# samson6460/tf2_YOLO

Hardware: AMD Instinct MI355X
Metric: images/sec training YOLOv3 416x416 bs=32/GPU (higher is better)
Workload: dtype f32-storage/fp16x2-mfma

## Files before the change

### include/yolo_hip.h

```cpp
#ifndef YOLO_HIP_H_
#define YOLO_HIP_H_

#include <stddef.h>
#include <stdint.h>

#ifdef __cplusplus
extern "C" {
#endif

typedef enum yolo_status {
  YOLO_OK = 0,
  YOLO_ERR_INVALID_ARG = -1,
  YOLO_ERR_LAUNCH = -2,
  YOLO_ERR_WORKSPACE = -3
} yolo_status;

enum { YOLO_ACT_LINEAR = 0, YOLO_ACT_LEAKY = 1, YOLO_ACT_MISH = 2 };
enum { YOLO_HEAD_V3 = 3, YOLO_HEAD_V2 = 2, YOLO_HEAD_V1 = 1, YOLO_HEAD_V4 = 4 };
enum { YOLO_NMS_HARD = 1, YOLO_NMS_SOFT = 2, YOLO_NMS_DIOU = 3 };

const char* yolo_last_error(void);
int yolo_abi_version(void);
int yolo_device_available(void);
int yolo_mfma_probe(const void* operands_f16, float* sink, int workgroups, int iters, double* flops_host, void* stream);

enum { YOLO_OPT_CONV_WIN = 0, YOLO_OPT_STAMPS = 1, YOLO_OPT_CONV_SK = 2, YOLO_OPT_CONV_PATCH = 5, YOLO_OPT_WGRAD_WIN = 6,
       YOLO_OPT_NMS_WALK = 7 ,
       YOLO_OPT_AB = 8  };
int yolo_set_option(int key, int value);
size_t yolo_conv_workspace_bytes(void);
int yolo_set_conv_workspace(void* p, size_t bytes, void* stream);
int yolo_set_debug_buffer(void* p, size_t bytes);

typedef struct yolo_conv_desc {
  int N, H, W, Cin;
  int Cout, kh, kw;
  int Ho, Wo;
  int sh, sw;
  int pad_t, pad_l;
} yolo_conv_desc;

#define YOLO_BN_STAT_SLOTS 64
#define YOLO_BN_RED_SLOTS 512
#define YOLO_SPLIT_BATCH_UNITS 4

int yolo_conv2d_fwd(const yolo_conv_desc* d, const float* x, const float* w,
                    const float* bias, float* y, double* stats, void* stream);
int yolo_conv2d_fwd_absmax(const yolo_conv_desc* d, const float* x, const float* w, const float* bias,
                           float* y, double* stats, unsigned* absmax, void* stream);

int yolo_conv2d_dgrad(const yolo_conv_desc* d, const float* dy, const float* wT,
// ... 237 lines not shown
```

### tf2_yolo_amd/csrc/conv_args.hpp

```cpp
#pragma once
#include "common.hpp"

namespace yolo {

constexpr int MAX_TAPS = 49;

struct Tap {
  int oy, ox, woff;
};

struct ClassGeom {
  long long M;
  int Hg, Wg, ooy, oox, tap0, ntaps;
};

struct GatherConvArgs {
  const float* src;
  const float* wgt;
  const float* bias;
  float* dst;
  double* stats;
  unsigned* absmax;
  long long M;
  int N, Hs, Ws, Cs;
// ... 7 lines not shown
  int tiles_n;
  int nblocks;
  unsigned src_bytes, wgt_bytes;
  int zero_blk_src, zero_blk_wgt;
  int nt_store;
  int vec_store;
  int kc;
  int dbg;
  const float* epi_scale;
  const float* epi_shift;
  const float* epi_res;
  int epi_act;
  unsigned char* out_planes;
  const float* pl_pred;
  const unsigned* pl_in_bound;
  const unsigned* pl_res_bound;
  int pl_in_n, pl_res_n;
  unsigned* pl_out_words;
  float* head_y;
  const float* head_anchors;
  int head_A, head_C;
  int sk_grid;
  int tile_order;
  float* sk_slabs;
  unsigned* sk_tickets;
  int split_parts;
  int ncls;
  ClassGeom cls[4];
  unsigned long long* stamps;
  const float* bwd_y;
  const float* bwd_scale;
  const float* bwd_shift;
  const float* bwd_mean;
  const float* bwd_invstd;
  float* bwd_part;
  unsigned* bwd_aux;
  int bwd_act;
  int bwd_nslots;
  int bwd_cap;
  Tap taps[MAX_TAPS];
};

#define YOLO_BNRED_CHECK(a)                                                                                          \
  if ((a).bwd_y != nullptr && (a).bwd_nslots > (a).bwd_cap) {                                                        \
    set_error("conv_dgrad(bn reduce): %d partial slots needed, room for %d", (a).bwd_nslots, (a).bwd_cap);           \
    return YOLO_ERR_INVALID_ARG;                                                                                     \
// ... 29 lines not shown

int launch_gather_split(GatherConvArgs& a, hipStream_t st);
bool gather_split_supported(const GatherConvArgs& a);
long long planes_bytes(long long rows, int C);
int launch_split_planes(const float* x, long long rows, int C, void* planes, hipStream_t st);
int launch_split_planes_absmax(const float* x, long long rows, int C, const unsigned* absmax, const float* extra_bound, int extra_n,
                               void* planes, float* out_bound, hipStream_t st);
int launch_split_planes_concat(const float* const* xs, const int* Cs, const float* const* bounds, int nsrc, long long rows,
                               void* planes, float* dst32, float* out_bound, hipStream_t st,
                               const int* bound_words = nullptr, const int* upsample = nullptr, int H = 0, int W = 0);
int launch_split_planes_padded(const float* x, long long rows, int Csrc, int C, void* planes, hipStream_t st);
int launch_split_planes_batch(const void* jobs, int njobs, long long total_blocks, hipStream_t st);
int launch_filter_transpose_batch(const void* jobs, int njobs, long long total_blocks, hipStream_t st);
int launch_gather_planes(GatherConvArgs& a, hipStream_t st);
bool conv_small_supported(const GatherConvArgs& a);
bool conv_small_head_supported(const GatherConvArgs& a);
int launch_conv_small(GatherConvArgs& a, hipStream_t st, int* nwg);
bool gather_planes_supported(const GatherConvArgs& a);
int conv_split_parts(const GatherConvArgs& a, long long nb, int bm, int min_cb, int idle_div);
int launch_split_reduce(GatherConvArgs& a, int bm, hipStream_t st);
float* conv_split_slabs();
int launch_conv_win(GatherConvArgs& a, int variant, hipStream_t st);
bool conv_win_supported(const GatherConvArgs& a);
enum { OPT_CONV_WIN = 0, OPT_STAMPS = 1, OPT_CONV_SK = 2, OPT_DBG = 3, OPT_TILE_ORDER = 4, OPT_CONV_PATCH = 5, OPT_WGRAD_WIN = 6, OPT_NMS_WALK = 7, OPT_EXP = 8, OPT_COUNT = 16 };
int set_conv_workspace(void* p, size_t bytes, hipStream_t st);
extern void* g_dbg_buf;
extern size_t g_dbg_bytes;
extern int g_opt[OPT_COUNT];
void init_options();
int launch_wgrad_planes(WgradArgs& a, hipStream_t st);
bool wgrad_planes_supported(const WgradArgs& a);
int launch_wgrad_win(WgradArgs& a, hipStream_t st);
bool wgrad_win_supported(const WgradArgs& a);
constexpr size_t WGRAD_WS_COLSUM_BYTES = 1 << 20;
void* wgrad_workspace(size_t* bytes);
bool stem_fwd_supported(const yolo_conv_desc* d);
struct StemEpiArgs {
  const float* scale;
  const float* shift;
  int act;
  void* planes;
  const float* pred;
  const unsigned* in_words;
  int in_n;
  unsigned* out_words;
};
bool stem_infer_supported(const yolo_conv_desc* d);
// ... 15 lines not shown
```

### tf2_yolo_amd/csrc/conv_win.hip

```cpp
#include "planes_epilogue.hpp"
#include <cstdlib>
#include <type_traits>

namespace yolo {

template <int WGM, int NCH, bool STAMPS = false, bool SPLIT = false, bool SK = false, int WGN = 2, int GEO = 0, bool BNRED = false>
__global__ __launch_bounds__(64 * WGM * WGN, 2) void conv_win_kernel(const GatherConvArgs a) {
  constexpr int BM = 64 * WGM, BN = 64 * WGN;
  constexpr int NW = WGM * WGN;
  constexpr int TM = 2, TN = 2;
  constexpr int NB = 4 * WGN / NW;
  constexpr int NWS = (NCH * 4) / NW;
  static_assert(NW == 4 || NW == 8, "4 or 8 waves");
  static_assert(NB == 1 || NB == 2, "filter loader roles: one (block, plane) or one block with both planes per wave");
  static_assert((NCH * 4) % NW == 0 && NWS <= 7, "window chunks: NCH*4 DMAs spread evenly, at most 7 stages");
  static_assert(GEO == 0 || (!SPLIT && !SK), "patch geometry: one workgroup per tile");
  constexpr int WIN_BYTES = NCH * 4096;
  constexpr int PLANE_STRIDE = 2 * NCH * 1024;
  constexpr int BSTAGE = 4096 * WGN;
  constexpr int BRING = 2 * WIN_BYTES;
  constexpr int LDS_TOTAL = 2 * WIN_BYTES + 3 * BSTAGE;
  constexpr int PH = BM / 16, PITCH = 18;
  static_assert(GEO == 0 || (PH + 2) * PITCH <= NCH * 64, "patch window does not fit the chunks");

  extern __shared__ __attribute__((aligned(16))) unsigned char smem[];
  const unsigned lds_base = (unsigned)(size_t)smem;

  const int tid = threadIdx.x;
  const int lane = tid & 63;
  const int wave = __builtin_amdgcn_readfirstlane(tid >> 6);
  const int wm = wave / WGN, wn = wave % WGN;
  [[maybe_unused]] unsigned long long stamp[4] = {0, 0, 0, 0}, phase_sum[3] = {0, 0, 0};
  auto take_stamp = [&](int i) {
    if constexpr (STAMPS) {
      __builtin_amdgcn_sched_barrier(0);
      stamp[i] = __builtin_amdgcn_s_memtime();
      __builtin_amdgcn_s_waitcnt(0xC07F);
      __builtin_amdgcn_sched_barrier(0);
    }
  };
  [[maybe_unused]] unsigned long long rt0 = 0, t_start = 0;
  [[maybe_unused]] int nparts_done = 0, epi_count = 0;
  [[maybe_unused]] unsigned long long epi_sum[6] = {0, 0, 0, 0, 0, 0};
  if constexpr (STAMPS) {
    rt0 = __builtin_amdgcn_s_memrealtime();
    t_start = __builtin_amdgcn_s_memtime();
  }

  const int H = a.Hs, W = a.Ws, P1 = GEO == 0 ? W + 1 : PITCH;
  const int HW = H * W;
  const int cpt = a.Cs >> 4;

  const i32x4 rsrcA = planes_rsrc(a.src, a.src_bytes), rsrcB = planes_rsrc(a.wgt, a.wgt_bytes);
  const unsigned blkstrideA = (unsigned)(cpt * PL_RECORD);
  const unsigned blkstrideB = (unsigned)((a.ldw >> 4) * PL_RECORD);
  int tapoff[9];
#pragma unroll
  for (int t = 0; t < 9; ++t) tapoff[t] = ((a.taps[t].oy + 1) * P1 + a.taps[t].ox + 1) * 16;

  const int G = (SK || SPLIT) ? a.sk_grid : 0;
  const int wl = xcd_remap(blockIdx.x, G > 0 ? G : a.nblocks);
  const int Gd = G > 0 ? G : 1;
  const int sk_q = G > 0 ? (a.nblocks * cpt) / Gd : 0, sk_r = G > 0 ? (a.nblocks * cpt) % Gd : 0;
  auto first_unit = [&](int w) { return w * sk_q + (w < sk_r ? w : sk_r); };
  const int sk_qd = sk_q > 0 ? sk_q : 1;
  auto owner_of = [&](int u) { return u < sk_r * (sk_q + 1) ? u / (sk_q + 1) : sk_r + (u - sk_r * (sk_q + 1)) / sk_qd; };
  const int SP = SPLIT ? a.split_parts : 1;
  const int u_begin = SPLIT ? (wl / SP) * cpt + ((wl % SP) * cpt) / SP : G > 0 ? first_unit(wl) : wl * cpt;
  const int u_end = SPLIT ? (wl / SP) * cpt + ((wl % SP + 1) * cpt) / SP : G > 0 ? first_unit(wl + 1) : (wl + 1) * cpt;

  for (int u_cur = u_begin; u_cur < u_end;) {
  take_stamp(0);
  const int tile = u_cur / cpt;
  const int cb0 = u_cur - tile * cpt;
  const int cb1 = (cpt - cb0 < u_end - u_cur) ? cpt : cb0 + (u_end - u_cur);
  u_cur += cb1 - cb0;
  const int tiles_m = a.nblocks / a.tiles_n;
  const int tile_n = a.tile_order ? tile / tiles_m : tile % a.tiles_n;
  const int tile_m = a.tile_order ? tile % tiles_m : tile / a.tiles_n;
  const long long m0 = (long long)tile_m * BM;
  const int n0 = tile_n * BN;
  [[maybe_unused]] int pn = 0, py0 = 0, px0 = 0;
  if constexpr (GEO == 1) {
    const int tx = (W + 15) >> 4, ty = (H + PH - 1) / PH;
    pn = tile_m / (tx * ty);
    const int rem = tile_m - pn * (tx * ty);
    py0 = (rem / tx) * PH;
    px0 = (rem % tx) * 16;
  }

  auto u_of = [&](long long m) -> int {
    const int n = (int)(m / HW);
    const int rem = (int)(m - (long long)n * HW);
    const int y = rem / W;
    return (n * (H + 1) + y + 1) * P1 + (rem - y * W) + 1;
  };
  const int u_m0 = GEO == 0 ? __builtin_amdgcn_readfirstlane(u_of(m0)) : 0;
  const int u_lo = u_m0 - P1 - 1;

  const int wplane = (wave >> 1) & 1, whf = wave & 1;
  unsigned voffW[NWS];
  int chunkW[NWS];
#pragma unroll
  for (int s = 0; s < NWS; ++s) {
    chunkW[s] = (NW == 4) ? s : 2 * s + (wave >> 2);
    const int u = u_lo + chunkW[s] * 64 + lane;
    unsigned v = (unsigned)a.zero_blk_src * blkstrideA;
    if constexpr (GEO == 1) {
      const int sl = chunkW[s] * 64 + lane;
      const int wy = sl / PITCH, wx = sl - wy * PITCH;
      const int sy = py0 - 1 + wy, sx = px0 - 1 + wx;
      if (wy < PH + 2 && (unsigned)sy < (unsigned)H && (unsigned)sx < (unsigned)W) {
        const int pix = (pn * H + sy) * W + sx;
        v = ((unsigned)pix >> 4) * blkstrideA + (unsigned)(pix & 15) * 16;
      }
    } else
    if (u >= 0) {
      const int vrow = u / P1, xc = u - vrow * P1;
      const int n = vrow / (H + 1), vr = vrow - n * (H + 1);
      if (xc >= 1 && vr >= 1 && n < a.N) {
        const int pix = (n * H + vr - 1) * W + xc - 1;
        v = ((unsigned)pix >> 4) * blkstrideA + (unsigned)(pix & 15) * 16;
      }
    }
    voffW[s] = v;
  }
  const unsigned soffW0 = (unsigned)(wplane * 512 + whf * 256);
  const unsigned ldsW0 = lds_base + (unsigned)((wplane * 2 + whf) * NCH * 1024);

  const int r = lane & 31, hf = lane >> 5;
  const int rbB = (NB == 2) ? wave : (wave >> 1);
  unsigned voffB;
  {
    const int co = n0 + rbB * 32 + r;
    const unsigned blk = co < a.Cout ? (unsigned)(co >> 4) : (unsigned)a.zero_blk_wgt;
    voffB = blk * blkstrideB + (co < a.Cout ? (unsigned)(co & 15) * 16 : 0u) + (unsigned)hf * 256;
  }

  unsigned abase[TM];
#pragma unroll
  for (int i = 0; i < TM; ++i) {
    const long long m = m0 + (wm * TM + i) * 32 + r;
    int wi;
    if constexpr (GEO == 1) {
      const int rr = (wm * TM + i) * 32 + r;
      wi = (rr >> 4) * PITCH + (rr & 15);
    } else {
      wi = (m < a.M) ? (u_of(m) - u_m0) : 0;
    }
    abase[i] = (unsigned)(hf * NCH * 1024 + wi * 16);
  }

  auto issue_window = [&](int s, int cb, int wb) {
    const int cbe = cb < cpt ? cb : cpt - 1;
    const unsigned so = __builtin_amdgcn_readfirstlane((unsigned)cbe * PL_RECORD + soffW0);
    const unsigned l = __builtin_amdgcn_readfirstlane(ldsW0 + (unsigned)(wb * WIN_BYTES + chunkW[s] * 1024));
    dma16(rsrcA, voffW[s], so, l);
  };
  auto issue_filter = [&](int d, int cb, int t, int rb3) {
    const int cbe = cb < cpt ? cb : cpt - 1;
    const int plane = (NB == 2) ? d : (wave & 1);
    const unsigned so = __builtin_amdgcn_readfirstlane((unsigned)(t * cpt + cbe) * PL_RECORD + (unsigned)plane * 512);
    const unsigned l = __builtin_amdgcn_readfirstlane(lds_base + (unsigned)(BRING + rb3 * BSTAGE + (rbB * 2 + plane) * 1024));
    dma16(rsrcB, voffB, so, l);
  };

  f32x16 acc[TM][TN];
#pragma unroll
  for (int i = 0; i < TM; ++i)
#pragma unroll
    for (int j = 0; j < TN; ++j)
#pragma unroll
      for (int q = 0; q < 16; ++q) acc[i][j][q] = 0.f;

  f16x8 fa[2][PL_PLANES][TM], fb[2][PL_PLANES][TN];
  auto read_frags = [&](int cb, auto T, auto SET) {
    constexpr int S = decltype(SET)::value;
    constexpr int t = decltype(T)::value;
    const unsigned so = (unsigned)((cb & 1) * WIN_BYTES + tapoff[t]);
    const unsigned char* sbB = smem + BRING + (t % 3) * BSTAGE + lane * 16;
#pragma unroll
    for (int p = 0; p < PL_PLANES; ++p) {
#pragma unroll
      for (int i = 0; i < TM; ++i)
        fa[S][p][i] = *reinterpret_cast<const f16x8*>(smem + (abase[i] + so) + p * PLANE_STRIDE);
#pragma unroll
      for (int j = 0; j < TN; ++j)
        fb[S][p][j] = *reinterpret_cast<const f16x8*>(sbB + ((wn * TN + j) * PL_PLANES + p) * 1024);
    }
  };

  auto mfma_stage = [&](int c, auto T, auto SET) {
    constexpr int S = decltype(SET)::value;
    constexpr int t = decltype(T)::value;
    constexpr int ND = NB + (t < NWS ? 1 : 0);
    constexpr int NM = TM * TN * 3;
    constexpr int t3 = (t + 3) % 9;
    const int c3 = c + (t + 3) / 9;
#pragma unroll
    for (int q = 0; q < 3; ++q) {
      const int pa = (q == 0) ? 1 : 0;
      const int pb = (q == 1) ? 1 : 0;
#pragma unroll
      for (int i = 0; i < TM; ++i)
#pragma unroll
        for (int j = 0; j < TN; ++j) {
          acc[i][j] = __builtin_amdgcn_mfma_f32_32x32x16_f16(fa[S][pa][i], fb[S][pb][j], acc[i][j], 0, 0, 0);
          const int idx = (q * TM + i) * TN + j;
#pragma unroll
          for (int d = 0; d < ND; ++d)
            if (idx == (((d + 1) * NM) / (ND + 1) > 0 ? ((d + 1) * NM) / (ND + 1) - 1 : 0)) {
              __builtin_amdgcn_sched_barrier(0);
              if (t < NWS && d == 0) issue_window(t, c + 1, (c + 1) & 1);
              else issue_filter(d - (t < NWS ? 1 : 0), c3, t3, t % 3);
              __builtin_amdgcn_sched_barrier(0);
            }
        }
    }
  };

#pragma unroll
  for (int s = 0; s < NWS; ++s) issue_window(s, cb0, cb0 & 1);
#pragma unroll
  for (int t = 0; t < 3; ++t)
#pragma unroll
    for (int d = 0; d < NB; ++d) issue_filter(d, cb0, t, t);
  asm volatile("s_waitcnt vmcnt(%0)" ::"n"(2 * NB) : "memory");
  __builtin_amdgcn_s_barrier();
  read_frags(cb0, std::integral_constant<int, 0>{}, std::integral_constant<int, 0>{});
  take_stamp(1);

  auto stage = [&](int c, auto T, auto SET) {
    constexpr int t = decltype(T)::value;
    constexpr int S = decltype(SET)::value;
    constexpr int wprev = (t >= 1 && t - 1 < NWS) ? 1 : 0;
    asm volatile("s_waitcnt vmcnt(%0)" ::"n"(NB + wprev) : "memory");
    asm volatile("s_waitcnt lgkmcnt(0)" ::: "memory");
    __builtin_amdgcn_s_barrier();
    constexpr int tn = (t + 1) % 9;
    read_frags(c + (t + 1) / 9, std::integral_constant<int, tn>{}, std::integral_constant<int, 1 - S>{});
    __builtin_amdgcn_sched_barrier(0);
    mfma_stage(c, T, SET);
  };
  auto block = [&](int c, auto P) {
    constexpr int p = decltype(P)::value;
    stage(c, std::integral_constant<int, 0>{}, std::integral_constant<int, (p + 0) & 1>{});
    stage(c, std::integral_constant<int, 1>{}, std::integral_constant<int, (p + 1) & 1>{});
    stage(c, std::integral_constant<int, 2>{}, std::integral_constant<int, (p + 2) & 1>{});
    stage(c, std::integral_constant<int, 3>{}, std::integral_constant<int, (p + 3) & 1>{});
    stage(c, std::integral_constant<int, 4>{}, std::integral_constant<int, (p + 4) & 1>{});
    stage(c, std::integral_constant<int, 5>{}, std::integral_constant<int, (p + 5) & 1>{});
    stage(c, std::integral_constant<int, 6>{}, std::integral_constant<int, (p + 6) & 1>{});
    stage(c, std::integral_constant<int, 7>{}, std::integral_constant<int, (p + 7) & 1>{});
    stage(c, std::integral_constant<int, 8>{}, std::integral_constant<int, (p + 8) & 1>{});
  };
  {
    int c = cb0;
    for (; c + 1 < cb1; c += 2) {
      block(c, std::integral_constant<int, 0>{});
      block(c + 1, std::integral_constant<int, 1>{});
    }
    if (c < cb1) block(c, std::integral_constant<int, 0>{});
  }
  take_stamp(2);
  asm volatile("s_waitcnt vmcnt(0)" ::: "memory");
  __syncthreads();

  bool finish = !SPLIT;
  if constexpr (SPLIT) store_split_slab<TM, TN>(a, acc, BM * BN * 4, wl, wave, lane);
  if constexpr (SK)
  if (cb1 - cb0 < cpt) {
    constexpr int SLAB_BYTES = BM * BN * 4;
    const int w_first = owner_of(tile * cpt), w_last = owner_of(tile * cpt + cpt - 1);
    const int nparts = w_last - w_first + 1;
    auto slab_of = [&](int w) {
      const int slot = (first_unit(w) / cpt == tile) ? 0 : 1;
      return reinterpret_cast<unsigned char*>(a.sk_slabs) + (size_t)(w * 2 + slot) * SLAB_BYTES;
    };
    {
      unsigned char* mine = slab_of(wl);
      const __amdgpu_buffer_rsrc_t rs = __builtin_amdgcn_make_buffer_rsrc(mine, 0, SLAB_BYTES, 0x00020000);
#pragma unroll
      for (int i = 0; i < TM; ++i)
#pragma unroll
        for (int j = 0; j < TN; ++j)
#pragma unroll
          for (int q4 = 0; q4 < 4; ++q4) {
            const f32x4 f = {acc[i][j][4 * q4], acc[i][j][4 * q4 + 1], acc[i][j][4 * q4 + 2], acc[i][j][4 * q4 + 3]};
            const u32x4 v = __builtin_bit_cast(u32x4, f);
            __builtin_amdgcn_raw_buffer_store_b128(v, rs, (((wave * TM + i) * TN + j) * 4 + q4) * 1024 + lane * 16, 0, 16 );
          }
    }
// ... 72 lines not shown
  }
  if constexpr (STAMPS) {
    const unsigned long long t_end = __builtin_amdgcn_s_memtime();
    const unsigned long long rt1 = __builtin_amdgcn_s_memrealtime();
    if (tid == 0 && a.stamps != nullptr) {
      unsigned long long* o = a.stamps + (size_t)blockIdx.x * 8;
      o[0] = t_start;
      o[1] = phase_sum[0];
      o[2] = phase_sum[1];
      o[3] = phase_sum[2];
      o[4] = t_end;
      o[5] = rt0;
      o[6] = rt1;
      o[7] = (unsigned long long)__builtin_amdgcn_s_getreg(((4 - 1) << 11) | (0 << 6) | 20) |
             ((unsigned long long)nparts_done << 8) | ((unsigned long long)gridDim.x << 32);
      unsigned long long* o2 = a.stamps + ((size_t)gridDim.x + blockIdx.x) * 8;
      for (int i = 0; i < 6; ++i) o2[i] = epi_sum[i];
      o2[6] = (unsigned long long)epi_count;
      o2[7] = 0;
    }
  }
}

static int win_pixels_needed(const GatherConvArgs& a, int BM) {
  const long long HW = (long long)a.Hs * a.Ws;
  const int P1 = a.Ws + 1;
  auto u_of = [&](long long m) -> long long {
    const long long n = m / HW, rem = m - n * HW;
    const long long y = rem / a.Ws;
    return (n * (a.Hs + 1) + y + 1) * P1 + (rem - y * a.Ws) + 1;
  };
  struct Key { long long M; int Hs, Ws, BM, need; };
  static thread_local Key cache[32];
  static thread_local int ncache = 0;
  for (int i = 0; i < ncache; ++i)
    if (cache[i].M == a.M && cache[i].Hs == a.Hs && cache[i].Ws == a.Ws && cache[i].BM == BM) return cache[i].need;
  long long worst = 0;
  for (long long m0 = 0; m0 < a.M; m0 += BM) {
    const long long ml = (m0 + BM - 1 < a.M) ? m0 + BM - 1 : a.M - 1;
    const long long need = u_of(ml) - u_of(m0) + 2 * P1 + 3;
    if (need > worst) worst = need;
  }
  if (ncache < 32) cache[ncache++] = Key{a.M, a.Hs, a.Ws, BM, (int)worst};
  return (int)worst;
}

bool conv_win_supported(const GatherConvArgs& a) {
  if (a.ntaps != 9 || a.sy != 1 || a.sx != 1 || a.Hg != a.Hs || a.Wg != a.Ws) return false;
  if ((a.Cs % 16) != 0 || a.Cout < 128 || a.ldw != 9 * a.Cs) return false;
  for (int t = 0; t < 9; ++t)
    if (a.taps[t].oy < -1 || a.taps[t].oy > 1 || a.taps[t].ox < -1 || a.taps[t].ox > 1 || a.taps[t].woff != t * a.Cs)
      return false;
  if ((long long)a.N * (a.Hs + 1) * (a.Ws + 1) + 2LL * a.Ws + 8 > 0x3fffffffLL) return false;
  return true;
}

constexpr size_t SK_TICKETS = 1 << 18;
static void* g_sk_ws = nullptr;
static size_t g_sk_bytes = 0;
int set_conv_workspace(void* p, size_t bytes, hipStream_t st) {
  g_sk_ws = nullptr;
  g_sk_bytes = 0;
  if (p == nullptr || bytes <= SK_TICKETS * 4) return YOLO_OK;
// ... 175 lines not shown
    if (hipGetDevice(&dev) != hipSuccess || hipDeviceGetAttribute(&cus, hipDeviceAttributeMultiprocessorCount, dev) != hipSuccess)
      cus = 256;
  }
  const long long slots = 2LL * cus;
  if (nb * idle_div > slots) return 1;
  long long P = (a.Cs >> 4) / min_cb;
  if (P > slots / nb) P = slots / nb;
  if (P > 32) P = 32;
  if (P < 2) return 1;
  if (SK_TICKETS * 4 + (size_t)(nb * P) * bm * 128 * 4 > g_sk_bytes) return 1;
  return (int)P;
}

int launch_split_reduce(GatherConvArgs& a, int bm, hipStream_t st) {
  if (bm == 128)
    hipLaunchKernelGGL(conv_split_reduce_kernel<128>, dim3((unsigned)a.nblocks * (128 * 128 / 4 / 256)), dim3(256), 0, st, a);
  else
    hipLaunchKernelGGL(conv_split_reduce_kernel<256>, dim3((unsigned)a.nblocks * (256 * 128 / 4 / 256)), dim3(256), 0, st, a);
  return check_launch("conv_split_reduce_kernel");
}

float* conv_split_slabs() { return reinterpret_cast<float*>(reinterpret_cast<unsigned char*>(g_sk_ws) + SK_TICKETS * 4); }

template <int WGM, int NCH>
static int launch_win(GatherConvArgs& a, hipStream_t st) {
  constexpr int BM = 64 * WGM;
  const long long tiles_m = (a.M + BM - 1) / BM;
  a.tiles_n = (a.Cout + 127) / 128;
  const long long nb = tiles_m * a.tiles_n;
  if (nb <= 0 || nb * (a.Cs >> 4) > 0x7fffffffLL) {
    set_error("conv(window): bad grid %lld", nb);
    return YOLO_ERR_INVALID_ARG;
  }
  a.nblocks = (int)nb;
  a.bwd_nslots = (int)tiles_m;
  YOLO_BNRED_CHECK(a)
  constexpr size_t lds = 2 * NCH * 4096 + 3 * 8192;
  static bool attr_set = false;
  static int resident = 0;
  if (!attr_set) {
    (void)hipFuncSetAttribute(reinterpret_cast<const void*>(&conv_win_kernel<WGM, NCH>),
                              hipFuncAttributeMaxDynamicSharedMemorySize, (int)lds);
    attr_set = true;
    int per_cu = 0, dev = 0, cus = 0;
    if (hipOccupancyMaxActiveBlocksPerMultiprocessor(&per_cu, reinterpret_cast<const void*>(&conv_win_kernel<WGM, NCH>),
                                                     128 * WGM, lds) == hipSuccess &&
        hipGetDevice(&dev) == hipSuccess &&
        hipDeviceGetAttribute(&cus, hipDeviceAttributeMultiprocessorCount, dev) == hipSuccess)
      resident = per_cu * cus;
  }
  {
    const long long wbytes = (long long)a.Cout * a.ldw * 4;
    a.tile_order = g_opt[OPT_TILE_ORDER] == 0 ? (wbytes >= (8LL << 20) ? 1 : 0) : g_opt[OPT_TILE_ORDER] - 1;
  }
  a.sk_grid = 0;
  a.dbg = g_opt[OPT_DBG];
  unsigned grid = (unsigned)nb;
  if (a.bwd_y != nullptr) {
    static bool attr_bn = false;
    if (!attr_bn) {
      (void)hipFuncSetAttribute(reinterpret_cast<const void*>(&conv_win_kernel<WGM, NCH, false, false, false, 2, 0, true>),
                                hipFuncAttributeMaxDynamicSharedMemorySize, (int)lds);
      attr_bn = true;
    }
    a.split_parts = 1;
    hipLaunchKernelGGL((conv_win_kernel<WGM, NCH, false, false, false, 2, 0, true>), dim3(grid), dim3(128 * WGM), lds, st, a);
    return check_launch("conv_win_kernel(bn reduce)");
  }
  static const int split_min_cb = [] { const char* e = getenv("YOLO_WIN_SPLIT_MIN_CB"); return e ? atoi(e) : 2; }();
  a.split_parts = WGM == 2 ? conv_split_parts(a, nb, BM, split_min_cb, 2) : 1;
  if (a.split_parts > 1) {
    a.tile_order = 0;
    a.sk_grid = (int)(nb * a.split_parts);
    a.sk_slabs = conv_split_slabs();
    if constexpr (WGM == 2) {
      static bool attr_split = false;
      if (!attr_split) {
        (void)hipFuncSetAttribute(reinterpret_cast<const void*>(&conv_win_kernel<WGM, NCH, false, true>),
                                  hipFuncAttributeMaxDynamicSharedMemorySize, (int)lds);
        attr_split = true;
      }
      hipLaunchKernelGGL((conv_win_kernel<WGM, NCH, false, true>), dim3((unsigned)a.sk_grid), dim3(128 * WGM), lds, st, a);
    }
    if (int rc = check_launch("conv_win_kernel(split)")) return rc;
    return launch_split_reduce(a, BM, st);
  }
  const bool sk_auto = g_opt[OPT_CONV_SK] == -1 && nb * 2 < resident && (a.Cs >> 4) >= 32;
  if ((sk_auto || g_opt[OPT_CONV_SK] > 1) && resident > 0 && g_sk_ws != nullptr && nb <= (long long)SK_TICKETS) {
    long long G = g_opt[OPT_CONV_SK] > 1 ? g_opt[OPT_CONV_SK] : resident;
    const long long units = nb * (a.Cs >> 4);
    if (sk_auto && G > nb * 4) G = nb * 4;
    if (G > units) G = units;
    if (SK_TICKETS * 4 + (size_t)G * 2 * BM * 128 * 4 <= g_sk_bytes && G >= 1) {
      a.sk_grid = (int)G;
      a.sk_tickets = reinterpret_cast<unsigned*>(g_sk_ws);
      a.sk_slabs = reinterpret_cast<float*>(reinterpret_cast<unsigned char*>(g_sk_ws) + SK_TICKETS * 4);
      grid = (unsigned)G;
    }
  }
  if constexpr (WGM == 2 && NCH == 5) {
    if (g_opt[OPT_STAMPS] != 0 && g_dbg_buf != nullptr && g_dbg_bytes >= (size_t)nb * 128) {
      static bool attr2 = false;
      if (!attr2) {
        (void)hipFuncSetAttribute(reinterpret_cast<const void*>(&conv_win_kernel<WGM, NCH, true>),
                                  hipFuncAttributeMaxDynamicSharedMemorySize, (int)lds);
        attr2 = true;
      }
      a.stamps = reinterpret_cast<unsigned long long*>(g_dbg_buf);
      hipLaunchKernelGGL((conv_win_kernel<WGM, NCH, true>), dim3(grid), dim3(128 * WGM), lds, st, a);
      return check_launch("conv_win_kernel(stamps)");
    }
  }
  if (a.sk_grid > 0) {
    static bool attr_sk = false;
    if (!attr_sk) {
      (void)hipFuncSetAttribute(reinterpret_cast<const void*>(&conv_win_kernel<WGM, NCH, false, false, true>),
                                hipFuncAttributeMaxDynamicSharedMemorySize, (int)lds);
      attr_sk = true;
    }
    hipLaunchKernelGGL((conv_win_kernel<WGM, NCH, false, false, true>), dim3(grid), dim3(128 * WGM), lds, st, a);
    return check_launch("conv_win_kernel(stream-K)");
  }
  hipLaunchKernelGGL((conv_win_kernel<WGM, NCH>), dim3(grid), dim3(128 * WGM), lds, st, a);
  return check_launch("conv_win_kernel");
}

static bool conv_patch_supported(const GatherConvArgs& a) {
  if (a.ntaps != 9 || a.sy != 1 || a.sx != 1 || a.Hg != a.Hs || a.Wg != a.Ws) return false;
  if (a.osy != 1 || a.osx != 1 || a.ooy != 0 || a.oox != 0 || a.Hd != a.Hg || a.Wd != a.Wg) return false;
  if ((a.Cs % 16) != 0 || a.Cout < 64 || a.ldw != 9 * a.Cs) return false;
  for (int t = 0; t < 9; ++t)
    if (a.taps[t].oy < -1 || a.taps[t].oy > 1 || a.taps[t].ox < -1 || a.taps[t].ox > 1 || a.taps[t].woff != t * a.Cs)
      return false;
  return true;
}

template <int WGM, int NCH, int WGN>
static int launch_patch(GatherConvArgs& a, hipStream_t st) {
  constexpr int BM = 64 * WGM, BN = 64 * WGN, PH = BM / 16;
  const long long tiles_m = (long long)a.N * ((a.Hg + PH - 1) / PH) * ((a.Wg + 15) / 16);
  a.tiles_n = (a.Cout + BN - 1) / BN;
  const long long nb = tiles_m * a.tiles_n;
  if (nb <= 0 || nb > 0x7fffffffLL) {
    set_error("conv(patch window): bad grid %lld", nb);
    return YOLO_ERR_INVALID_ARG;
  }
  a.nblocks = (int)nb;
  a.bwd_nslots = (int)tiles_m;
  YOLO_BNRED_CHECK(a)
  constexpr size_t lds = 2 * NCH * 4096 + 3 * 4096 * WGN;
  auto kern = &conv_win_kernel<WGM, NCH, false, false, false, WGN, 1>;
  static bool attr_set = false;
  if (!attr_set) {
    (void)hipFuncSetAttribute(reinterpret_cast<const void*>(kern), hipFuncAttributeMaxDynamicSharedMemorySize, (int)lds);
    attr_set = true;
  }
  a.tile_order = 0;
  a.sk_grid = 0;
  a.split_parts = 1;
  a.dbg = g_opt[OPT_DBG];
  if (a.bwd_y != nullptr) {
    auto kern_bn = &conv_win_kernel<WGM, NCH, false, false, false, WGN, 1, true>;
    static bool attr_bn = false;
    if (!attr_bn) {
      (void)hipFuncSetAttribute(reinterpret_cast<const void*>(kern_bn), hipFuncAttributeMaxDynamicSharedMemorySize, (int)lds);
      attr_bn = true;
    }
    hipLaunchKernelGGL(kern_bn, dim3((unsigned)nb), dim3(64 * WGM * WGN), lds, st, a);
    return check_launch("conv_win_kernel(patch, bn reduce)");
  }
  hipLaunchKernelGGL(kern, dim3((unsigned)nb), dim3(64 * WGM * WGN), lds, st, a);
  return check_launch("conv_win_kernel(patch)");
}

static int launch_conv_patch(GatherConvArgs& a, hipStream_t st) {
  const int mode = g_opt[OPT_CONV_PATCH];
  if (mode == 0 || !conv_patch_supported(a)) return 1;
  const bool narrow = a.Cout <= 64;
  if (mode == 1) {
    if (!narrow && a.Ws <= 64) return 1;
    const long long tiles = narrow ? (long long)a.N * ((a.Hg + 15) / 16) * ((a.Wg + 15) / 16)
                                   : (long long)a.N * ((a.Hg + 7) / 8) * ((a.Wg + 15) / 16) * ((a.Cout + 127) / 128);
    if (tiles < 256) return 1;
  }
  return narrow ? launch_patch<4, 6, 1>(a, st) : launch_patch<2, 3, 2>(a, st);
}

int launch_conv_win(GatherConvArgs& a, int variant, hipStream_t st) {
  if (variant != 2 && variant != 4) {
    const int rc = launch_conv_patch(a, st);
    if (rc <= 0) return rc;
  }
  if (!conv_win_supported(a)) return 1;
  int wgm = variant;
  if (wgm != 2 && wgm != 4) {
    if (a.Ws > 64) return 1;
    wgm = 2;
  }
  const int need = win_pixels_needed(a, 64 * wgm);
  const int nch = (need + 63) / 64;
  if (wgm == 2) {
    switch (nch) {
      case 1: case 2: case 3: return launch_win<2, 3>(a, st);
      case 4: return launch_win<2, 4>(a, st);
      case 5: return launch_win<2, 5>(a, st);
      case 6: return launch_win<2, 6>(a, st);
      case 7: return launch_win<2, 7>(a, st);
      default: return 1;
    }
  }
  switch ((nch + 1) / 2) {
    case 1: case 2: return launch_win<4, 4>(a, st);
    case 3: return launch_win<4, 6>(a, st);
    case 4: return launch_win<4, 8>(a, st);
    case 5: return launch_win<4, 10>(a, st);
    case 6: return launch_win<4, 12>(a, st);
    case 7: return launch_win<4, 14>(a, st);
    default: return 1;
  }
}

}
```

### tf2_yolo_amd/csrc/runtime.hip

```cpp
#include "conv_args.hpp"
#include <cstdlib>
#include <cstring>

namespace yolo {

static thread_local char g_err[512] = "";

void set_error(const char* fmt, ...) {
  va_list ap;
  va_start(ap, fmt);
  vsnprintf(g_err, sizeof(g_err), fmt, ap);
  va_end(ap);
}

int g_opt[OPT_COUNT];
void* g_dbg_buf = nullptr;
size_t g_dbg_bytes = 0;
static void options_from_env() {
  for (int i = 0; i < OPT_COUNT; ++i) g_opt[i] = 0;
  const char* e = getenv("YOLO_CONV_WIN");
  g_opt[OPT_CONV_WIN] = e ? atoi(e) : 1;
  e = getenv("YOLO_CONV_SK");
  g_opt[OPT_CONV_SK] = e ? atoi(e) : 1;
  e = getenv("YOLO_CONV_PATCH");
  g_opt[OPT_CONV_PATCH] = e ? atoi(e) : 1;
  e = getenv("YOLO_WGRAD_WIN");
  g_opt[OPT_WGRAD_WIN] = e ? atoi(e) : 1;
  e = getenv("YOLO_NMS_WALK");
  g_opt[OPT_NMS_WALK] = e ? atoi(e) : 0;
  e = getenv("YOLO_EXP");
  g_opt[OPT_EXP] = e ? atoi(e) : 0;
}
void init_options() {
  static bool done = false;
  if (done) return;
  done = true;
  options_from_env();
}

}

extern "C" int yolo_set_option(int key, int value) {
  yolo::init_options();
  if (key == -1) {
    yolo::options_from_env();
    return YOLO_OK;
  }
  if (key < 0 || key >= yolo::OPT_COUNT) {
    yolo::set_error("yolo_set_option: unknown key %d", key);
    return YOLO_ERR_INVALID_ARG;
  }
  yolo::g_opt[key] = value;
// ... 56 lines not shown
```

### tf2_yolo_amd/ops.py

```python
import ctypes
from ctypes import byref, c_void_p

import torch

from . import _lib
from . import tape as _tape
from ._lib import ConvDesc, LossCfg, YoloHipError, check

BN_EPS = 1e-3
BN_MOMENTUM = 0.99
BN_STAT_SLOTS = 64
BN_RED_SLOTS = 512
SPLIT_BATCH_UNITS = 4


class KernelTimer:

    def __init__(self):
        self.pending = []

    def bracket(self, name, flops, launches, fn, layer=None):
        s, e = torch.cuda.Event(enable_timing=True), torch.cuda.Event(enable_timing=True)
        s.record()
        fn()
# ... 95 lines not shown
def _win_key(d, hs, ws, cs):
    if d.kh == 3 and d.kw == 3 and d.sh == 1 and d.sw == 1 and d.pad_t == 1 and d.pad_l == 1 and cs % 16 == 0 \
            and d.H == d.Ho and d.W == d.Wo:
        return (ws, d.N * hs * ws, hs, d.N)
    return None


def _gather_variant(cout, flat, m=None):
    bn = 32 if cout <= 32 else (64 if cout <= 64 else 128)
    bm = 128
    if bn == 128 and not flat and m is not None and ((m + 127) // 128) * ((cout + 127) // 128) <= 512:
        bm = 64
    if CONV_MODE == "split" and not flat and cout > 32:
        waves = {(128, 64): "2,2", (64, 128): "1,4", (128, 128): "4,2"}[(bm, bn)]
        return f"gather_conv_split_kernel<{bm},{bn},{waves}>"
    return f"gather_conv_kernel<{bm},{bn}{',flat' if flat else ''}>"


OPT_CONV_WIN = 0
OPT_CONV_SK = 2
OPT_CONV_PATCH = 5
OPT_WGRAD_WIN = 6
OPT_NMS_WALK = 7
_CONV_WS = None


def ensure_conv_workspace():
    global _CONV_WS
    if _CONV_WS is not None and _CONV_WS.device.index != torch.cuda.current_device():
        raise YoloHipError(f"libyolo_hip.so was initialised on cuda:{_CONV_WS.device.index} and cannot also serve "
                           f"cuda:{torch.cuda.current_device()}: start one process per GPU")
    if _CONV_WS is None:
        lib = _lib.load()
        n = int(lib.yolo_conv_workspace_bytes())
        _CONV_WS = torch.empty(n, dtype=torch.uint8, device="cuda")
        check(lib.yolo_set_conv_workspace(_p(_CONV_WS), n, _stream()), "yolo_set_conv_workspace")
    return _CONV_WS


_WGRAD_WS = None


def ensure_wgrad_workspace():
    global _WGRAD_WS
    if _WGRAD_WS is None:
        lib = _lib.load()
# ... 1004 lines not shown
```

Baseline: 1074.

## Add unpadded window geometry with per-tap masking and banded tile ordering for conv_win

Adds a new window geometry (GEO=2), on by default, that addresses the unpadded activation planes directly, with pitch W and row u equal to m. Halo correctness comes from a per-row 9-bit tap mask that zeroes out-of-bounds A fragments after each LDS read. This shrinks the per-tile window and drops the padded-index arithmetic, at the cost of extra select instructions in the MFMA loop. It also adds a banded tile-order mode for split launches, picking a band height that minimises the A+B bytes touched per wave of workgroups, and changes how split parts map to slabs.

After: 1073, median of 2. Within noise of the previous version (-0.1%).

```diff
diff --git a/include/yolo_hip.h b/include/yolo_hip.h
--- a/include/yolo_hip.h
+++ b/include/yolo_hip.h
@@ -26,7 +26,9 @@
 
 enum { YOLO_OPT_CONV_WIN = 0, YOLO_OPT_STAMPS = 1, YOLO_OPT_CONV_SK = 2, YOLO_OPT_CONV_PATCH = 5, YOLO_OPT_WGRAD_WIN = 6,
        YOLO_OPT_NMS_WALK = 7 ,
-       YOLO_OPT_AB = 8  };
+       YOLO_OPT_AB = 8 ,
+       YOLO_OPT_TILE_ORDER = 4 ,
+       YOLO_OPT_WIN_GEO = 9  };
 int yolo_set_option(int key, int value);
 size_t yolo_conv_workspace_bytes(void);
 int yolo_set_conv_workspace(void* p, size_t bytes, void* stream);
diff --git a/tf2_yolo_amd/csrc/conv_args.hpp b/tf2_yolo_amd/csrc/conv_args.hpp
--- a/tf2_yolo_amd/csrc/conv_args.hpp
+++ b/tf2_yolo_amd/csrc/conv_args.hpp
@@ -53,6 +53,7 @@
   int head_A, head_C;
   int sk_grid;
   int tile_order;
+  int tile_band;
   float* sk_slabs;
   unsigned* sk_tickets;
   int split_parts;
@@ -128,7 +129,7 @@
 float* conv_split_slabs();
 int launch_conv_win(GatherConvArgs& a, int variant, hipStream_t st);
 bool conv_win_supported(const GatherConvArgs& a);
-enum { OPT_CONV_WIN = 0, OPT_STAMPS = 1, OPT_CONV_SK = 2, OPT_DBG = 3, OPT_TILE_ORDER = 4, OPT_CONV_PATCH = 5, OPT_WGRAD_WIN = 6, OPT_NMS_WALK = 7, OPT_EXP = 8, OPT_COUNT = 16 };
+enum { OPT_CONV_WIN = 0, OPT_STAMPS = 1, OPT_CONV_SK = 2, OPT_DBG = 3, OPT_TILE_ORDER = 4, OPT_CONV_PATCH = 5, OPT_WGRAD_WIN = 6, OPT_NMS_WALK = 7, OPT_EXP = 8, OPT_WIN_GEO = 9, OPT_COUNT = 16 };
 int set_conv_workspace(void* p, size_t bytes, hipStream_t st);
 extern void* g_dbg_buf;
 extern size_t g_dbg_bytes;
diff --git a/tf2_yolo_amd/csrc/conv_win.hip b/tf2_yolo_amd/csrc/conv_win.hip
--- a/tf2_yolo_amd/csrc/conv_win.hip
+++ b/tf2_yolo_amd/csrc/conv_win.hip
@@ -1,4 +1,5 @@
 #include "planes_epilogue.hpp"
+#include "win_geom.hpp"
 #include <cstdlib>
 #include <type_traits>
 
@@ -14,14 +15,14 @@
   static_assert(NW == 4 || NW == 8, "4 or 8 waves");
   static_assert(NB == 1 || NB == 2, "filter loader roles: one (block, plane) or one block with both planes per wave");
   static_assert((NCH * 4) % NW == 0 && NWS <= 7, "window chunks: NCH*4 DMAs spread evenly, at most 7 stages");
-  static_assert(GEO == 0 || (!SPLIT && !SK), "patch geometry: one workgroup per tile");
+  static_assert(GEO != 1 || (!SPLIT && !SK), "patch geometry: one workgroup per tile");
   constexpr int WIN_BYTES = NCH * 4096;
   constexpr int PLANE_STRIDE = 2 * NCH * 1024;
   constexpr int BSTAGE = 4096 * WGN;
   constexpr int BRING = 2 * WIN_BYTES;
   constexpr int LDS_TOTAL = 2 * WIN_BYTES + 3 * BSTAGE;
   constexpr int PH = BM / 16, PITCH = 18;
-  static_assert(GEO == 0 || (PH + 2) * PITCH <= NCH * 64, "patch window does not fit the chunks");
+  static_assert(GEO != 1 || (PH + 2) * PITCH <= NCH * 64, "patch window does not fit the chunks");
 
   extern __shared__ __attribute__((aligned(16))) unsigned char smem[];
   const unsigned lds_base = (unsigned)(size_t)smem;
@@ -47,16 +48,19 @@
     t_start = __builtin_amdgcn_s_memtime();
   }
 
-  const int H = a.Hs, W = a.Ws, P1 = GEO == 0 ? W + 1 : PITCH;
-  const int HW = H * W;
+  const int H = a.Hs, W = a.Ws, P1 = win_pitch(GEO, W);
   const int cpt = a.Cs >> 4;
 
   const i32x4 rsrcA = planes_rsrc(a.src, a.src_bytes), rsrcB = planes_rsrc(a.wgt, a.wgt_bytes);
   const unsigned blkstrideA = (unsigned)(cpt * PL_RECORD);
   const unsigned blkstrideB = (unsigned)((a.ldw >> 4) * PL_RECORD);
-  int tapoff[9];
-#pragma unroll
-  for (int t = 0; t < 9; ++t) tapoff[t] = ((a.taps[t].oy + 1) * P1 + a.taps[t].ox + 1) * 16;
+  int tapoff[9], toy[9], tox[9];
+#pragma unroll
+  for (int t = 0; t < 9; ++t) {
+    toy[t] = a.taps[t].oy;
+    tox[t] = a.taps[t].ox;
+    tapoff[t] = ((toy[t] + 1) * P1 + tox[t] + 1) * 16;
+  }
 
   const int G = (SK || SPLIT) ? a.sk_grid : 0;
   const int wl = xcd_remap(blockIdx.x, G > 0 ? G : a.nblocks);
@@ -66,8 +70,10 @@
   const int sk_qd = sk_q > 0 ? sk_q : 1;
   auto owner_of = [&](int u) { return u < sk_r * (sk_q + 1) ? u / (sk_q + 1) : sk_r + (u - sk_r * (sk_q + 1)) / sk_qd; };
   const int SP = SPLIT ? a.split_parts : 1;
-  const int u_begin = SPLIT ? (wl / SP) * cpt + ((wl % SP) * cpt) / SP : G > 0 ? first_unit(wl) : wl * cpt;
-  const int u_end = SPLIT ? (wl / SP) * cpt + ((wl % SP + 1) * cpt) / SP : G > 0 ? first_unit(wl + 1) : (wl + 1) * cpt;
+  const int sp_tile = (SPLIT && a.tile_order == 2) ? wl % a.nblocks : wl / SP;
+  const int sp_part = (SPLIT && a.tile_order == 2) ? wl / a.nblocks : wl % SP;
+  const int u_begin = SPLIT ? sp_tile * cpt + (sp_part * cpt) / SP : G > 0 ? first_unit(wl) : wl * cpt;
+  const int u_end = SPLIT ? sp_tile * cpt + ((sp_part + 1) * cpt) / SP : G > 0 ? first_unit(wl + 1) : (wl + 1) * cpt;
 
   for (int u_cur = u_begin; u_cur < u_end;) {
   take_stamp(0);
@@ -76,8 +82,8 @@
   const int cb1 = (cpt - cb0 < u_end - u_cur) ? cpt : cb0 + (u_end - u_cur);
   u_cur += cb1 - cb0;
   const int tiles_m = a.nblocks / a.tiles_n;
-  const int tile_n = a.tile_order ? tile / tiles_m : tile % a.tiles_n;
-  const int tile_m = a.tile_order ? tile % tiles_m : tile / a.tiles_n;
+  int tile_m, tile_n;
+  win_tile_coords(tile, tiles_m, a.tiles_n, a.tile_order, a.tile_band, &tile_m, &tile_n);
   const long long m0 = (long long)tile_m * BM;
   const int n0 = tile_n * BN;
   [[maybe_unused]] int pn = 0, py0 = 0, px0 = 0;
@@ -89,13 +95,7 @@
     px0 = (rem % tx) * 16;
   }
 
-  auto u_of = [&](long long m) -> int {
-    const int n = (int)(m / HW);
-    const int rem = (int)(m - (long long)n * HW);
-    const int y = rem / W;
-    return (n * (H + 1) + y + 1) * P1 + (rem - y * W) + 1;
-  };
-  const int u_m0 = GEO == 0 ? __builtin_amdgcn_readfirstlane(u_of(m0)) : 0;
+  const int u_m0 = GEO != 1 ? __builtin_amdgcn_readfirstlane(win_u(GEO, m0, H, W)) : 0;
   const int u_lo = u_m0 - P1 - 1;
 
   const int wplane = (wave >> 1) & 1, whf = wave & 1;
@@ -114,6 +114,8 @@
         const int pix = (pn * H + sy) * W + sx;
         v = ((unsigned)pix >> 4) * blkstrideA + (unsigned)(pix & 15) * 16;
       }
+    } else if constexpr (GEO == 2) {
+      if (u >= 0 && (long long)u < a.M) v = ((unsigned)u >> 4) * blkstrideA + (unsigned)(u & 15) * 16;
     } else
     if (u >= 0) {
       const int vrow = u / P1, xc = u - vrow * P1;
@@ -138,17 +140,12 @@
   }
 
   unsigned abase[TM];
+  [[maybe_unused]] unsigned tmask[TM];
 #pragma unroll
   for (int i = 0; i < TM; ++i) {
-    const long long m = m0 + (wm * TM + i) * 32 + r;
-    int wi;
-    if constexpr (GEO == 1) {
-      const int rr = (wm * TM + i) * 32 + r;
-      wi = (rr >> 4) * PITCH + (rr & 15);
-    } else {
-      wi = (m < a.M) ? (u_of(m) - u_m0) : 0;
-    }
-    abase[i] = (unsigned)(hf * NCH * 1024 + wi * 16);
+    const int rr = (wm * TM + i) * 32 + r;
+    abase[i] = (unsigned)(hf * NCH * 1024 + win_row_slot(GEO, m0, rr, a.M, H, W) * 16);
+    if constexpr (GEO == 2) tmask[i] = win_tap_mask(m0 + rr, H, W, toy, tox);
   }
 
   auto issue_window = [&](int s, int cb, int wb) {
@@ -190,6 +187,18 @@
     }
   };
 
+  auto mask_frags = [&](auto T, auto SET) {
+    constexpr int S = decltype(SET)::value;
+    constexpr int t = decltype(T)::value;
+    const f16x8 z = {};
+#pragma unroll
+    for (int i = 0; i < TM; ++i) {
+      const bool in = (tmask[i] & (1u << t)) != 0;
+#pragma unroll
+      for (int p = 0; p < PL_PLANES; ++p) fa[S][p][i] = in ? fa[S][p][i] : z;
+    }
+  };
+
   auto mfma_stage = [&](int c, auto T, auto SET) {
     constexpr int S = decltype(SET)::value;
     constexpr int t = decltype(T)::value;
@@ -228,6 +237,7 @@
   asm volatile("s_waitcnt vmcnt(%0)" ::"n"(2 * NB) : "memory");
   __builtin_amdgcn_s_barrier();
   read_frags(cb0, std::integral_constant<int, 0>{}, std::integral_constant<int, 0>{});
+  if constexpr (GEO == 2) mask_frags(std::integral_constant<int, 0>{}, std::integral_constant<int, 0>{});
   take_stamp(1);
 
   auto stage = [&](int c, auto T, auto SET) {
@@ -241,6 +251,10 @@
     read_frags(c + (t + 1) / 9, std::integral_constant<int, tn>{}, std::integral_constant<int, 1 - S>{});
     __builtin_amdgcn_sched_barrier(0);
     mfma_stage(c, T, SET);
+    if constexpr (GEO == 2) {
+      __builtin_amdgcn_sched_barrier(0);
+      mask_frags(std::integral_constant<int, tn>{}, std::integral_constant<int, 1 - S>{});
+    }
   };
   auto block = [&](int c, auto P) {
     constexpr int p = decltype(P)::value;
@@ -267,7 +281,7 @@
   __syncthreads();
 
   bool finish = !SPLIT;
-  if constexpr (SPLIT) store_split_slab<TM, TN>(a, acc, BM * BN * 4, wl, wave, lane);
+  if constexpr (SPLIT) store_split_slab<TM, TN>(a, acc, BM * BN * 4, (tile_m * a.tiles_n + tile_n) * SP + sp_part, wave, lane);
   if constexpr (SK)
   if (cb1 - cb0 < cpt) {
     constexpr int SLAB_BYTES = BM * BN * 4;
@@ -386,14 +400,8 @@
   }
 }
 
-static int win_pixels_needed(const GatherConvArgs& a, int BM) {
-  const long long HW = (long long)a.Hs * a.Ws;
-  const int P1 = a.Ws + 1;
-  auto u_of = [&](long long m) -> long long {
-    const long long n = m / HW, rem = m - n * HW;
-    const long long y = rem / a.Ws;
-    return (n * (a.Hs + 1) + y + 1) * P1 + (rem - y * a.Ws) + 1;
-  };
+static int win_pixels_needed(const GatherConvArgs& a, int BM, int geo) {
+  if (geo == 2) return (int)win_tile_need(2, 0, BM, a.M, a.Hs, a.Ws);
   struct Key { long long M; int Hs, Ws, BM, need; };
   static thread_local Key cache[32];
   static thread_local int ncache = 0;
@@ -401,8 +409,7 @@
     if (cache[i].M == a.M && cache[i].Hs == a.Hs && cache[i].Ws == a.Ws && cache[i].BM == BM) return cache[i].need;
   long long worst = 0;
   for (long long m0 = 0; m0 < a.M; m0 += BM) {
-    const long long ml = (m0 + BM - 1 < a.M) ? m0 + BM - 1 : a.M - 1;
-    const long long need = u_of(ml) - u_of(m0) + 2 * P1 + 3;
+    const long long need = win_tile_need(0, m0, BM, a.M, a.Hs, a.Ws);
     if (need > worst) worst = need;
   }
   if (ncache < 32) cache[ncache++] = Key{a.M, a.Hs, a.Ws, BM, (int)worst};
@@ -624,7 +631,24 @@
 
 float* conv_split_slabs() { return reinterpret_cast<float*>(reinterpret_cast<unsigned char*>(g_sk_ws) + SK_TICKETS * 4); }
 
-template <int WGM, int NCH>
+static void win_tile_order(GatherConvArgs& a, long long nb, int P, int BM) {
+  const long long wbytes = (long long)a.Cout * a.ldw * 4;
+  const int opt = g_opt[OPT_TILE_ORDER];
+  a.tile_band = 1;
+  if (opt == -1) {
+    a.tile_order = (P == 1 && wbytes >= (8LL << 20)) ? 1 : 0;
+  } else if (opt == 1 || opt == 2) {
+    a.tile_order = opt - 1;
+  } else if (opt == 0 && P == 1) {
+    a.tile_order = wbytes >= (8LL << 20) ? 1 : 0;
+  } else {
+    const int tiles_m = (int)(nb / a.tiles_n);
+    a.tile_order = 2;
+    a.tile_band = win_band(tiles_m, a.tiles_n, (nb * P + 7) / 8, (double)BM * a.Cs * 4, 128.0 * a.ldw * 4);
+  }
+}
+
+template <int WGM, int NCH, int GEO>
 static int launch_win(GatherConvArgs& a, hipStream_t st) {
   constexpr int BM = 64 * WGM;
   const long long tiles_m = (a.M + BM - 1) / BM;
@@ -641,48 +665,45 @@
   static bool attr_set = false;
   static int resident = 0;
   if (!attr_set) {
-    (void)hipFuncSetAttribute(reinterpret_cast<const void*>(&conv_win_kernel<WGM, NCH>),
+    (void)hipFuncSetAttribute(reinterpret_cast<const void*>(&conv_win_kernel<WGM, NCH, false, false, false, 2, GEO>),
                               hipFuncAttributeMaxDynamicSharedMemorySize, (int)lds);
     attr_set = true;
     int per_cu = 0, dev = 0, cus = 0;
-    if (hipOccupancyMaxActiveBlocksPerMultiprocessor(&per_cu, reinterpret_cast<const void*>(&conv_win_kernel<WGM, NCH>),
+    if (hipOccupancyMaxActiveBlocksPerMultiprocessor(&per_cu, reinterpret_cast<const void*>(&conv_win_kernel<WGM, NCH, false, false, false, 2, GEO>),
                                                      128 * WGM, lds) == hipSuccess &&
         hipGetDevice(&dev) == hipSuccess &&
         hipDeviceGetAttribute(&cus, hipDeviceAttributeMultiprocessorCount, dev) == hipSuccess)
       resident = per_cu * cus;
   }
-  {
-    const long long wbytes = (long long)a.Cout * a.ldw * 4;
-    a.tile_order = g_opt[OPT_TILE_ORDER] == 0 ? (wbytes >= (8LL << 20) ? 1 : 0) : g_opt[OPT_TILE_ORDER] - 1;
-  }
+  win_tile_order(a, nb, 1, BM);
   a.sk_grid = 0;
   a.dbg = g_opt[OPT_DBG];
   unsigned grid = (unsigned)nb;
   if (a.bwd_y != nullptr) {
     static bool attr_bn = false;
     if (!attr_bn) {
-      (void)hipFuncSetAttribute(reinterpret_cast<const void*>(&conv_win_kernel<WGM, NCH, false, false, false, 2, 0, true>),
+      (void)hipFuncSetAttribute(reinterpret_cast<const void*>(&conv_win_kernel<WGM, NCH, false, false, false, 2, GEO, true>),
                                 hipFuncAttributeMaxDynamicSharedMemorySize, (int)lds);
       attr_bn = true;
     }
     a.split_parts = 1;
-    hipLaunchKernelGGL((conv_win_kernel<WGM, NCH, false, false, false, 2, 0, true>), dim3(grid), dim3(128 * WGM), lds, st, a);
+    hipLaunchKernelGGL((conv_win_kernel<WGM, NCH, false, false, false, 2, GEO, true>), dim3(grid), dim3(128 * WGM), lds, st, a);
     return check_launch("conv_win_kernel(bn reduce)");
   }
   static const int split_min_cb = [] { const char* e = getenv("YOLO_WIN_SPLIT_MIN_CB"); return e ? atoi(e) : 2; }();
   a.split_parts = WGM == 2 ? conv_split_parts(a, nb, BM, split_min_cb, 2) : 1;
   if (a.split_parts > 1) {
-    a.tile_order = 0;
+    win_tile_order(a, nb, a.split_parts, BM);
     a.sk_grid = (int)(nb * a.split_parts);
     a.sk_slabs = conv_split_slabs();
     if constexpr (WGM == 2) {
       static bool attr_split = false;
       if (!attr_split) {
-        (void)hipFuncSetAttribute(reinterpret_cast<const void*>(&conv_win_kernel<WGM, NCH, false, true>),
+        (void)hipFuncSetAttribute(reinterpret_cast<const void*>(&conv_win_kernel<WGM, NCH, false, true, false, 2, GEO>),
                                   hipFuncAttributeMaxDynamicSharedMemorySize, (int)lds);
         attr_split = true;
       }
-      hipLaunchKernelGGL((conv_win_kernel<WGM, NCH, false, true>), dim3((unsigned)a.sk_grid), dim3(128 * WGM), lds, st, a);
+      hipLaunchKernelGGL((conv_win_kernel<WGM, NCH, false, true, false, 2, GEO>), dim3((unsigned)a.sk_grid), dim3(128 * WGM), lds, st, a);
     }
     if (int rc = check_launch("conv_win_kernel(split)")) return rc;
     return launch_split_reduce(a, BM, st);
@@ -700,7 +721,7 @@
       grid = (unsigned)G;
     }
   }
-  if constexpr (WGM == 2 && NCH == 5) {
+  if constexpr (WGM == 2 && NCH == 5 && GEO == 0) {
     if (g_opt[OPT_STAMPS] != 0 && g_dbg_buf != nullptr && g_dbg_bytes >= (size_t)nb * 128) {
       static bool attr2 = false;
       if (!attr2) {
@@ -716,14 +737,14 @@
   if (a.sk_grid > 0) {
     static bool attr_sk = false;
     if (!attr_sk) {
-      (void)hipFuncSetAttribute(reinterpret_cast<const void*>(&conv_win_kernel<WGM, NCH, false, false, true>),
+      (void)hipFuncSetAttribute(reinterpret_cast<const void*>(&conv_win_kernel<WGM, NCH, false, false, true, 2, GEO>),
                                 hipFuncAttributeMaxDynamicSharedMemorySize, (int)lds);
       attr_sk = true;
     }
-    hipLaunchKernelGGL((conv_win_kernel<WGM, NCH, false, false, true>), dim3(grid), dim3(128 * WGM), lds, st, a);
+    hipLaunchKernelGGL((conv_win_kernel<WGM, NCH, false, false, true, 2, GEO>), dim3(grid), dim3(128 * WGM), lds, st, a);
     return check_launch("conv_win_kernel(stream-K)");
   }
-  hipLaunchKernelGGL((conv_win_kernel<WGM, NCH>), dim3(grid), dim3(128 * WGM), lds, st, a);
+  hipLaunchKernelGGL((conv_win_kernel<WGM, NCH, false, false, false, 2, GEO>), dim3(grid), dim3(128 * WGM), lds, st, a);
   return check_launch("conv_win_kernel");
 }
 
@@ -758,6 +779,7 @@
     attr_set = true;
   }
   a.tile_order = 0;
+  a.tile_band = 1;
   a.sk_grid = 0;
   a.split_parts = 1;
   a.dbg = g_opt[OPT_DBG];
@@ -788,6 +810,31 @@
   return narrow ? launch_patch<4, 6, 1>(a, st) : launch_patch<2, 3, 2>(a, st);
 }
 
+template <int GEO>
+static int launch_conv_win_geo(GatherConvArgs& a, int wgm, hipStream_t st) {
+  const int need = win_pixels_needed(a, 64 * wgm, GEO);
+  const int nch = (need + 63) / 64;
+  if (wgm == 2) {
+    switch (nch) {
+      case 1: case 2: case 3: return launch_win<2, 3, GEO>(a, st);
+      case 4: return launch_win<2, 4, GEO>(a, st);
+      case 5: return launch_win<2, 5, GEO>(a, st);
+      case 6: return launch_win<2, 6, GEO>(a, st);
+      case 7: return launch_win<2, 7, GEO>(a, st);
+      default: return 1;
+    }
+  }
+  switch ((nch + 1) / 2) {
+    case 1: case 2: return launch_win<4, 4, GEO>(a, st);
+    case 3: return launch_win<4, 6, GEO>(a, st);
+    case 4: return launch_win<4, 8, GEO>(a, st);
+    case 5: return launch_win<4, 10, GEO>(a, st);
+    case 6: return launch_win<4, 12, GEO>(a, st);
+    case 7: return launch_win<4, 14, GEO>(a, st);
+    default: return 1;
+  }
+}
+
 int launch_conv_win(GatherConvArgs& a, int variant, hipStream_t st) {
   if (variant != 2 && variant != 4) {
     const int rc = launch_conv_patch(a, st);
@@ -799,27 +846,8 @@
     if (a.Ws > 64) return 1;
     wgm = 2;
   }
-  const int need = win_pixels_needed(a, 64 * wgm);
-  const int nch = (need + 63) / 64;
-  if (wgm == 2) {
-    switch (nch) {
-      case 1: case 2: case 3: return launch_win<2, 3>(a, st);
-      case 4: return launch_win<2, 4>(a, st);
-      case 5: return launch_win<2, 5>(a, st);
-      case 6: return launch_win<2, 6>(a, st);
-      case 7: return launch_win<2, 7>(a, st);
-      default: return 1;
-    }
-  }
-  switch ((nch + 1) / 2) {
-    case 1: case 2: return launch_win<4, 4>(a, st);
-    case 3: return launch_win<4, 6>(a, st);
-    case 4: return launch_win<4, 8>(a, st);
-    case 5: return launch_win<4, 10>(a, st);
-    case 6: return launch_win<4, 12>(a, st);
-    case 7: return launch_win<4, 14>(a, st);
-    default: return 1;
-  }
-}
-
-}
+  if (g_opt[OPT_WIN_GEO] == 0) return launch_conv_win_geo<0>(a, wgm, st);
+  return launch_conv_win_geo<2>(a, wgm, st);
+}
+
+}
diff --git a/tf2_yolo_amd/csrc/runtime.hip b/tf2_yolo_amd/csrc/runtime.hip
--- a/tf2_yolo_amd/csrc/runtime.hip
+++ b/tf2_yolo_amd/csrc/runtime.hip
@@ -28,6 +28,10 @@
   g_opt[OPT_WGRAD_WIN] = e ? atoi(e) : 1;
   e = getenv("YOLO_NMS_WALK");
   g_opt[OPT_NMS_WALK] = e ? atoi(e) : 0;
+  e = getenv("YOLO_WIN_GEO");
+  g_opt[OPT_WIN_GEO] = e ? atoi(e) : 2;
+  e = getenv("YOLO_TILE_ORDER");
+  g_opt[OPT_TILE_ORDER] = e ? atoi(e) : 0;
   e = getenv("YOLO_EXP");
   g_opt[OPT_EXP] = e ? atoi(e) : 0;
 }
diff --git a/tf2_yolo_amd/csrc/win_geom.hpp b/tf2_yolo_amd/csrc/win_geom.hpp
--- /dev/null
+++ b/tf2_yolo_amd/csrc/win_geom.hpp
@@ -0,0 +1,79 @@
+#pragma once
+#if defined(__HIPCC__) || defined(__HIP__)
+#define WIN_HD __host__ __device__ __forceinline__
+#else
+#define WIN_HD inline
+#endif
+
+namespace yolo {
+
+constexpr int WIN_PATCH_PITCH = 18;
+
+WIN_HD int win_pitch(int geo, int W) { return geo == 0 ? W + 1 : geo == 2 ? W : WIN_PATCH_PITCH; }
+
+WIN_HD int win_u(int geo, long long m, int H, int W) {
+  if (geo == 2) return (int)m;
+  const long long HW = (long long)H * W;
+  const int n = (int)(m / HW);
+  const int rem = (int)(m - (long long)n * HW);
+  const int y = rem / W;
+  return (n * (H + 1) + y + 1) * (W + 1) + (rem - y * W) + 1;
+}
+
+WIN_HD int win_row_slot(int geo, long long m0, int rr, long long M, int H, int W) {
+  if (geo == 1) return (rr >> 4) * WIN_PATCH_PITCH + (rr & 15);
+  if (geo == 2) return rr;
+  const long long m = m0 + rr;
+  return m < M ? win_u(0, m, H, W) - win_u(0, m0, H, W) : 0;
+}
+
+WIN_HD long long win_tile_need(int geo, long long m0, int BM, long long M, int H, int W) {
+  const int P = win_pitch(geo, W);
+  if (geo == 2) return (long long)BM + 2 * P + 2;
+  const long long ml = (m0 + BM - 1 < M) ? m0 + BM - 1 : M - 1;
+  return (long long)win_u(0, ml, H, W) - win_u(0, m0, H, W) + 2 * P + 3;
+}
+
+WIN_HD unsigned win_tap_mask(long long m, int H, int W, const int* oy, const int* ox) {
+  const long long HW = (long long)H * W;
+  const int rem = (int)(m - (m / HW) * HW);
+  const int y = rem / W, x = rem - (rem / W) * W;
+  unsigned bits = 0;
+  for (int t = 0; t < 9; ++t)
+    if ((unsigned)(y + oy[t]) < (unsigned)H && (unsigned)(x + ox[t]) < (unsigned)W) bits |= 1u << t;
+  return bits;
+}
+
+WIN_HD void win_tile_coords(int tile, int tiles_m, int tiles_n, int order, int band, int* tm, int* tn) {
+  if (order == 0) {
+    *tn = tile % tiles_n;
+    *tm = tile / tiles_n;
+  } else if (order == 1) {
+    *tn = tile / tiles_m;
+    *tm = tile % tiles_m;
+  } else {
+    const int b0 = (tile / (band * tiles_n)) * band;
+    const int hb = (tiles_m - b0 < band) ? tiles_m - b0 : band;
+    const int idx = tile - b0 * tiles_n;
+    *tn = idx / hb;
+    *tm = b0 + idx % hb;
+  }
+}
+
+inline int win_band(int tiles_m, int tiles_n, long long run, double a_row, double b_col) {
+  int best = tiles_m;
+  double best_b = -1.0;
+  for (int h = tiles_m; h >= 1; --h) {
+    long long w = (run + h - 1) / h;
+    if (w > tiles_n) break;
+    const long long hh = run < h ? run : h;
+    const double b = (double)hh * a_row + (double)w * b_col;
+    if (best_b < 0.0 || b < best_b) {
+      best_b = b;
+      best = h;
+    }
+  }
+  return best;
+}
+
+}
diff --git a/tf2_yolo_amd/ops.py b/tf2_yolo_amd/ops.py
--- a/tf2_yolo_amd/ops.py
+++ b/tf2_yolo_amd/ops.py
@@ -141,6 +141,8 @@
 OPT_CONV_PATCH = 5
 OPT_WGRAD_WIN = 6
 OPT_NMS_WALK = 7
+OPT_TILE_ORDER = 4
+OPT_WIN_GEO = 9
 _CONV_WS = None
 
 
```
